# slcs-jsc/mptrac

Hardware: AMD Instinct MI355X
Metric: particle-steps/s (higher is better)
Workload: dtype f64

## Files before the change

### mptrac_amd/csrc/mphip_api.hip

```cpp
#include <hip/hip_runtime.h>
#include <dlfcn.h>
#include <unistd.h>

#include <algorithm>
#include <atomic>
#include <cmath>
#include <cstdio>
#include <cstring>
#include <string>
#include <mutex>
#include <thread>
#include <vector>

#include "mphip_kernels.hpp"
#include "mphip_metprep.hpp"
#include "mphip_regrid.hpp"
#include "mphip_detrend.hpp"

using namespace mphip;

namespace {

constexpr unsigned kAdv = MPHIP_MOD_TIMESTEPS | MPHIP_MOD_POSITION | MPHIP_MOD_ADVECT | MPHIP_MOD_POSITION2;
constexpr unsigned kAdvTurb = kAdv | MPHIP_MOD_DIFF_TURB;
constexpr unsigned kAdvDiff = kAdvTurb | MPHIP_MOD_DIFF_MESO;
constexpr unsigned kAdvTurbConvSedi = kAdvTurb | MPHIP_MOD_CONVECTION | MPHIP_MOD_SEDI;
constexpr unsigned kAdvDiffConvSedi = kAdvDiff | MPHIP_MOD_CONVECTION | MPHIP_MOD_SEDI;
constexpr unsigned kDiffConvSediOnly = MPHIP_MOD_TIMESTEPS | MPHIP_MOD_DIFF_TURB | MPHIP_MOD_DIFF_MESO | MPHIP_MOD_CONVECTION
  | MPHIP_MOD_SEDI | MPHIP_MOD_POSITION2;
constexpr unsigned kTailOnly = MPHIP_MOD_TIMESTEPS;
constexpr unsigned kBound = MPHIP_MOD_BOUND_COND | MPHIP_MOD_BOUND_COND2;
constexpr unsigned kParticleBits = 0x3fffu | MPHIP_MOD_ISOSURF | kBound | MPHIP_MOD_ISOSURF_INIT;

struct MetSlot {
  bool valid = false;
  double time = 0;
  float *f3[MPHIP_N3D] = {};
  float *f2[MPHIP_N2D] = {};
  bool has3[MPHIP_N3D] = {};
  bool has2[MPHIP_N2D] = {};
  std::vector<double> lon, lat, p;
  float ps11 = 0.f;
  double ps_min = -HUGE_VAL, pct_min = -HUGE_VAL;
  double ps_max = HUGE_VAL, pbl_min = -HUGE_VAL, pbl_max = HUGE_VAL, pel_min = -HUGE_VAL;
};

}

struct mphip_ctx {
  int device = 0;
  hipStream_t stream = nullptr;
  std::string err;
  std::mutex err_lock;

  mphip_ctl_t ctl;
  bool have_ctl = false;
  DevClim *d_clim = nullptr;
  bool have_clim = false;
  double *d_zm[MPHIP_NZM] = {};
  DevZm zm[MPHIP_NZM] = {};
  double *d_ts[MPHIP_NTR] = {};
  DevTracerSeries h_tracers = {};
  DevTracerSeries *d_tracers = nullptr;

  MetSlot slot[2];
  int flip = 0;
  MetSlot next;
  bool next_pending = false;
  hipStream_t copy_stream = nullptr;
  hipEvent_t next_ready = nullptr;
  hipEvent_t main_mark = nullptr;
  bool fuse_sort = true;
  const int *fused_perm = nullptr;
  bool fuse_quantities = true;
  bool fused_quantities = false;
  const int *fold_perm = nullptr;
  bool lazy_meteo = true;
  bool meteo_pending = false;
  bool pin_host_atm = false;
  std::vector<std::pair<uintptr_t, uintptr_t>> pinned;
  std::mutex pinned_lock;
  std::thread uploader;
  int uploader_rc = 0;
  std::atomic<bool> uploader_done{ false };
  std::string uploader_err;
  int nx = 0, ny = 0, npl = 0, coord_type = 0;
  int nml = 0;
  struct PackedGrids {
    float *wind = nullptr, *temp = nullptr, *h2o = nullptr;
    float *mlw = nullptr, *zl2 = nullptr, *pl2 = nullptr;
    f32x4 *mx = nullptr, *mx2 = nullptr;
    f32x4 *cloud = nullptr, *sfa = nullptr, *sfb = nullptr, *sfc = nullptr, *sfd = nullptr;
    f32x4 *cp2 = nullptr;
    int *ml_mono = nullptr;
    bool ml_monotonic = false;
    float *meso = nullptr;
    bool meso_valid = false;
    void release() {
      for (void *q : { (void *) wind, (void *) temp, (void *) h2o, (void *) mlw, (void *) zl2, (void *) pl2, (void *) mx,
                       (void *) mx2, (void *) cloud, (void *) sfa, (void *) sfb, (void *) sfc, (void *) sfd, (void *) cp2,
                       (void *) ml_mono, (void *) meso })
        if (q)
          (void) hipFree(q);
      *this = PackedGrids();
    }
  };
  PackedGrids pk, pk_next;
  bool pk_next_valid = false;
  std::vector<double> h_lon, h_lat, h_p;
  double *d_axes = nullptr;
  int lut_base = 0, lut_size = 0;
  size_t axes_bytes = 0;
  bool packed_dirty = true;

  long long np = 0, ip0 = 0, np_total = 0, cap = 0;
  int nq = 0;
  double *d_arr[4 + MPHIP_NQ_MAX] = {};
  double *d_alt[4 + MPHIP_NQ_MAX] = {};
  float *d_uvwp[3] = {};
  float *d_uvwp_alt[3] = {};
  double *d_dt = nullptr;
  double *d_dt_alt = nullptr;
  uint64_t rng_ctr = 0;
  double *d_iso = nullptr, *d_iso_alt = nullptr;
  int *d_kz = nullptr, *d_kz_alt = nullptr;
  double *d_iso_ts = nullptr, *d_iso_ps = nullptr;
  int iso_n = 0;

  int *d_ext = nullptr, *d_ext_alt = nullptr;
  bool ext_identity = true;
  int locality_interval = 60;
  double *d_rec = nullptr;
  size_t rec_cap = 0;
  bool grid_records = true;
  int chain_blocks = 0;
  double *h_sums = nullptr;
  size_t h_sums_cap = 0;
  double *d_grid_kernel = nullptr;
  double *d_ana_kernel = nullptr;
  size_t ana_kernel_cap = 0;
  uint32_t *d_marks = nullptr;
  size_t marks_cap = 0;
  int *d_slot_of = nullptr;
  size_t slot_of_cap = 0;
  uint32_t *d_ana_flags = nullptr;
  int grid_nk = 0;
  bool locality_zorder = false;
  int locality_tile = 0;
  int step_blocks = 8192;
  int step_blocks_multi = 32768;
  int xcd_map = 1;
  int big_grid = 0;
  int perm_records = 1;
  void *d_prec = nullptr;
  size_t prec_cap = 0;
  int multi_step = 64;
  bool fold_resort = true;
  bool force_generic = false;
  bool compact_depo = true;
  int sort_bits = 0;
  int steps_since_resort = 1 << 30;

  uint32_t *d_keys[2] = {};
  int *d_vals[2] = {};
  uint32_t *d_counts = nullptr;
  size_t counts_cap = 0;
  int sorted_buf = -1;
  int lds_tile = 0;
  bool emit_keys = true;
  unsigned char *d_depo_busy = nullptr;
  long long depo_busy_cap = 0;
  bool told_shortcuts_off = false;
  bool depo_busy_valid = false;
  bool sort_repair = true;
  bool ahead_priority = false;
  bool stored_is_sorted = false;
  long long sorted_n = 0;
  uint32_t *rep_sk = nullptr, *rep_mk[2] = {}, *rep_fk = nullptr, *rep_tiles = nullptr, *rep_nm = nullptr;
  int *rep_si = nullptr, *rep_mi[2] = {}, *rep_fv = nullptr;
  long long rep_cap = 0;
  bool sort_ahead = true;
  bool ahead_box = true;
  hipStream_t ahead_stream = nullptr;
  hipEvent_t ahead_mark = nullptr, ahead_done = nullptr;
  uint32_t *ahead_keys[2] = {};
  int *ahead_vals[2] = {};
  uint32_t *ahead_counts = nullptr;
  size_t ahead_counts_cap = 0;
  double *ahead_dt = nullptr;
  long long ahead_cap = 0;
  bool ahead_valid = false;
  double ahead_t = 0;
  int ahead_cur = 0;

  int *d_cell = nullptr;
  double *d_sums = nullptr;
  size_t sums_cap = 0;

  int *d_cnt = nullptr;
  double *d_chemgrid = nullptr;
  bool chemgrid_ok = false;
  double h2o2_low = 0;
  double *d_photo = nullptr;
  DevPhoto photo = {};
  bool photo_have[4] = {};
  RadioQnt radio = { { -1, -1, -1, -1, -1, -1 } };
  bool radio_on = false;
  bool rdepo_on = false;
  mphip_box_t rdepo_grid = {};
  double *d_rdepo_inv = nullptr;
// ... 77 lines not shown
    (void) hipFree(p);
}

int grid_for(long long n, int block = 256, int maxb = 8192) {
  long long b = (n + block - 1) / block;
  if (b < 1)
    b = 1;
  if (b > maxb)
    b = maxb;
  return (int) b;
}

DevAtm dev_atm(const mphip_ctx *c) {
  DevAtm a;
  a.time = c->d_arr[0];
  a.p = c->d_arr[1];
  a.lon = c->d_arr[2];
  a.lat = c->d_arr[3];
  for (int iq = 0; iq < MPHIP_NQ_MAX; iq++)
    a.q[iq] = iq < c->nq ? c->d_arr[4 + iq] : nullptr;
  a.up = c->d_uvwp[0];
  a.vp = c->d_uvwp[1];
  a.wp = c->d_uvwp[2];
  a.dt = c->d_dt;
  a.ext = c->ext_identity ? nullptr : c->d_ext;
  a.iso = c->d_iso;
  a.kz = c->d_kz;
  a.iso_ts = c->d_iso_ts;
  a.iso_ps = c->d_iso_ps;
  a.iso_n = c->iso_n;
  a.perm = c->fold_perm ? c->fold_perm : c->fused_perm;
  a.s_time = c->d_alt[0];
  a.s_p = c->d_alt[1];
  a.s_lon = c->d_alt[2];
  a.s_lat = c->d_alt[3];
  a.nq_perm = c->fold_perm || (c->fused_perm && c->fused_quantities) ? c->nq : 0;
  a.perm_all = c->fold_perm ? 1 : 0;
  a.s_up = c->d_uvwp_alt[0];
  a.s_vp = c->d_uvwp_alt[1];
  a.s_wp = c->d_uvwp_alt[2];
  a.s_dt = c->d_dt_alt;
  a.s_ext = c->d_ext_alt;
  a.ext_out = c->d_ext;
  for (int iq = 0; iq < MPHIP_NQ_MAX; iq++)
    a.s_q[iq] = iq < c->nq ? c->d_alt[4 + iq] : nullptr;
  a.np = c->np;
  a.ip0 = c->ip0;
  a.np_total = c->np_total;
  return a;
}

static bool weights_stay_inside(int coord_type, double first, double last) {
  return coord_type != 0 || (last - first >= 360.0 && first <= 0.0 && first >= -360.0);
}

DevMet dev_met(const mphip_ctx *c) {
  DevMet M;
  M.wind = c->pk.wind;
  M.temp = c->pk.temp;
  M.cloud = c->pk.cloud;
  M.mx = c->pk.mx;
  M.mx2 = c->pk.mx2;
  M.sfa = c->pk.sfa;
  M.sfb = c->pk.sfb;
  M.cp2 = c->pk.cp2;
  M.sfc = c->pk.sfc;
  M.sfd = c->pk.sfd;
  M.h2o = c->pk.h2o;
  M.mlw = c->pk.mlw;
  M.zl2 = c->pk.zl2;
  M.pl2 = c->pk.pl2;
  M.meso = c->pk.meso_valid ? c->pk.meso : nullptr;
  M.meso_nty = (c->ny + 2) / 4;
  M.ml_monotonic = c->pk.ml_monotonic ? 1 : 0;
  for (int t = 0; t < 2; t++) {
    M.zl[t] = c->slot[t ^ c->flip].f3[MPHIP_ZETAL];
    M.pll[t] = c->slot[t ^ c->flip].f3[MPHIP_PL];
  }
  M.npl = c->nml;
  M.axes = c->d_axes;
  M.lut_base = c->lut_base;
  M.lut_size = c->lut_size;
  M.lat_x0 = c->h_lat[0];
  M.lat_inv_dx = (c->ny - 1) / (c->h_lat[c->ny - 1] - c->h_lat[0]);
  M.nx = c->nx;
  M.ny = c->ny;
  M.np = c->npl;
  M.coord_type = c->coord_type;
  M.time0 = c->slot[0 ^ c->flip].time;
  M.time1 = c->slot[1 ^ c->flip].time;
  M.inv_dtime = 1.0 / (M.time1 - M.time0);
  double latmin = c->h_lat[0], latmax = c->h_lat[0];
  for (double v : c->h_lat) {
    latmin = std::min(latmin, v);
    latmax = std::max(latmax, v);
  }
  M.latmin = latmin;
  M.latmax = latmax;
  M.local = (std::fabs(c->h_lon[c->nx - 1] - c->h_lon[0] - 360.0) >= 0.01);
  const int my = (c->ny - 1) >> 1, mp = (c->npl - 1) >> 1;
  M.lat_ascending = c->h_lat[my] < c->h_lat[my + 1];
  M.p_ascending = c->h_p[mp] < c->h_p[mp + 1];
  M.lon_first = c->h_lon[0];
  M.lon_last = c->h_lon[c->nx - 1];
  M.inv_dlon0 = 1.0 / (c->h_lon[1] - c->h_lon[0]);
  M.lat_search_max = std::nextafter(latmax, -HUGE_VAL);
  M.p_min = *std::min_element(c->h_p.begin(), c->h_p.end());
  M.p_search_max = std::nextafter(*std::max_element(c->h_p.begin(), c->h_p.end()), -HUGE_VAL);
  M.p_cmp_off = M.p_ascending ? 1 : 0;
  M.p_step = M.p_ascending ? 1 : -1;
  M.ps11[0] = c->slot[0 ^ c->flip].ps11;
  M.ps11[1] = c->slot[1 ^ c->flip].ps11;
  M.ps_skip = std::min(c->slot[0].ps_min, c->slot[1].ps_min) - 1e-6;
  M.pct_skip = std::min(c->slot[0].pct_min, c->slot[1].pct_min) - 1e-6;
  {
    const double ps_lo = std::min(c->slot[0].ps_min, c->slot[1].ps_min), ps_hi = std::max(c->slot[0].ps_max, c->slot[1].ps_max);
    const double pbl_lo = std::min(c->slot[0].pbl_min, c->slot[1].pbl_min),
                 pbl_hi = std::max(c->slot[0].pbl_max, c->slot[1].pbl_max);
    auto p1_min = [&](double trans) {
      double lo = HUGE_VAL;
      for (double pbl : { pbl_lo, pbl_hi })
        for (double ps : { ps_lo, ps_hi })
          lo = std::min(lo, pbl - trans * (ps - pbl));
      return lo;
    };
    const bool known = std::isfinite(ps_lo) && std::isfinite(ps_hi) && std::isfinite(pbl_lo) && std::isfinite(pbl_hi);
    M.turb_skip = -HUGE_VAL;
    M.conv_skip = -HUGE_VAL;
    if (known && c->have_ctl) {
      const double b = std::min({ ps_lo, pbl_lo, p1_min(c->ctl.turb_pbl_trans) });
      M.turb_skip = b - 1e-6 * std::fabs(b) - 1e-6;
      double lo = ps_lo;
      if (c->ctl.conv_mix_pbl)
        lo = std::min(lo, p1_min(c->ctl.conv_pbl_trans));
      if (c->ctl.conv_cape >= 0)
        lo = std::min(lo, std::min(c->slot[0].pel_min, c->slot[1].pel_min));
      if (lo == lo)
        M.conv_skip = lo - 1e-6 * std::fabs(lo) - 1e-6;
    }
  }
  if (!weights_stay_inside(c->coord_type, c->h_lon[0], c->h_lon[c->nx - 1]))
    M.ps_skip = M.pct_skip = M.turb_skip = M.conv_skip = -HUGE_VAL;
  M.meso_dt = std::fabs(c->ctl.dt_mod);
  M.meso_r = 1 - 2 * M.meso_dt / c->ctl.dt_met;
  M.meso_r2 = std::sqrt(1 - M.meso_r * M.meso_r);
  if (!c->have_ctl || !(M.meso_dt > 0) || !std::isfinite(M.meso_r2))
    M.meso_dt = -1;
  return M;
}

size_t axes_lds_bytes(const mphip_ctx *c) {
  return c->axes_bytes;
}

int host_locate_irr(const std::vector<double> &xx, double x) {
  const int n = (int) xx.size();
  int lo = 0, hi = n - 1;
  int mid = (hi + lo) >> 1;
  if (xx[mid] < xx[mid + 1]) {
    while (hi > lo + 1) {
      mid = (hi + lo) >> 1;
      if (xx[mid] > x)
        hi = mid;
      else
        lo = mid;
    }
  } else {
    while (hi > lo + 1) {
      mid = (hi + lo) >> 1;
      if (xx[mid] <= x)
        hi = mid;
      else
        lo = mid;
    }
  }
  return lo;
}

int upload_axes(mphip_ctx *ctx) {
  const int nx = ctx->nx, ny = ctx->ny, np = ctx->npl;
  const size_t nd = 2 * (size_t) (nx + ny + np);
  std::vector<int16_t> lut;
  ctx->lut_base = ctx->lut_size = 0;
  const double pmin = *std::min_element(ctx->h_p.begin(), ctx->h_p.end());
  const double pmax = *std::max_element(ctx->h_p.begin(), ctx->h_p.end());
  if (pmin > 0 && std::isfinite(pmax) && np < 32000) {
    long long kmin, kmax;
    memcpy(&kmin, &pmin, 8);
    memcpy(&kmax, &pmax, 8);
    kmin >>= 45;
    kmax >>= 45;
    if (kmax - kmin + 1 <= 8192) {
      ctx->lut_base = (int) kmin;
      ctx->lut_size = (int) (kmax - kmin + 1);
      lut.resize((size_t) ctx->lut_size);
// ... 2570 lines not shown
    const int nx = ctl->chemgrid_nx, ny = ctl->chemgrid_ny, nz = ctl->chemgrid_nz;
    const double dz = (ctl->chemgrid_z1 - ctl->chemgrid_z0) / nz;
    const double dlon = (ctl->chemgrid_lon1 - ctl->chemgrid_lon0) / nx;
    const double dlat = (ctl->chemgrid_lat1 - ctl->chemgrid_lat0) / ny;
    std::vector<double> tab((size_t) nz + 2 * (size_t) ny + nx);
    double *press = tab.data(), *area = press + nz, *lon = area + ny, *lat = lon + nx;
    for (int iz = 0; iz < nz; iz++)
      press[iz] = kP0 * exp(-(ctl->chemgrid_z0 + dz * (iz + 0.5)) / kH0);
    for (int ix = 0; ix < nx; ix++)
      lon[ix] = ctl->chemgrid_lon0 + dlon * (ix + 0.5);
    for (int iy = 0; iy < ny; iy++) {
      lat[iy] = ctl->chemgrid_lat0 + dlat * (iy + 0.5);
      area[iy] = dlat * dlon * ((kRE * M_PI / 180.) * (kRE * M_PI / 180.)) * cos(lat[iy] * M_PI / 180.);
    }
    HIPCHK(hipSetDevice(ctx->device));
    HIPCHK(hipStreamSynchronize(ctx->stream));
    if (dev_alloc(ctx, &ctx->d_chemgrid, tab.size()))
      return 1;
    HIPCHK(hipMemcpy(ctx->d_chemgrid, tab.data(), tab.size() * sizeof(double), hipMemcpyHostToDevice));
    ctx->chemgrid_ok = true;
  }
  ctx->h2o2_low = pow(1. / kH2O2CorA, 1. / kH2O2CorB);
  ctx->ctl = *ctl;
  ctx->have_ctl = true;
  return 0;
}

int mphip_update_clim(mphip_ctx *ctx, int ntime, int nlat, const double *tropo_time, const double *tropo_lat,
                      const double *tropo, int ld) {
  if (!ctx || !tropo_time || !tropo_lat || !tropo)
    return fail(ctx, "null argument");
  if (ntime < 2 || ntime > 12 || nlat < 2 || nlat > 73 || ld < nlat)
    return fail(ctx, "tropopause climatology dimensions out of range");
  HIPCHK(hipSetDevice(ctx->device));
  DevClim h;
  memset(&h, 0, sizeof(h));
  h.ntime = ntime;
  h.nlat = nlat;
  for (int i = 0; i < ntime; i++)
    h.time[i] = tropo_time[i];
  for (int j = 0; j < nlat; j++)
    h.lat[j] = tropo_lat[j];
  for (int i = 0; i < ntime; i++)
    for (int j = 0; j < nlat; j++)
      h.tropo[i][j] = tropo[(size_t) i * ld + j];
  for (int i = 0; i + 1 < ntime; i++)
    h.inv_dtime[i] = 1.0 / (h.time[i + 1] - h.time[i]);
  for (int j = 0; j + 1 < nlat; j++)
    h.inv_dlat[j] = 1.0 / (h.lat[j + 1] - h.lat[j]);
  if (!ctx->d_clim)
    HIPCHK(hipMalloc((void **) &ctx->d_clim, sizeof(DevClim)));
  HIPCHK(hipMemcpyAsync(ctx->d_clim, &h, sizeof(DevClim), hipMemcpyHostToDevice, ctx->stream));
  HIPCHK(hipStreamSynchronize(ctx->stream));
  ctx->have_clim = true;
  return 0;
}

int mphip_update_clim_zm(mphip_ctx *ctx, int which, int ntime, int np, int nlat, const double *time, const double *p,
                         const double *lat, const double *vmr) {
  if (!ctx || which < 0 || which >= MPHIP_NZM)
    return fail(ctx, "bad argument");
  HIPCHK(hipSetDevice(ctx->device));
  if (flush_meteo(ctx))
    return 1;
  HIPCHK(hipStreamSynchronize(ctx->stream));
  dev_free(ctx->d_zm[which]);
  ctx->d_zm[which] = nullptr;
  memset(&ctx->zm[which], 0, sizeof(DevZm));
  if (ntime == 0)
    return 0;
  if (!time || !p || !lat || !vmr)
    return fail(ctx, "null argument");
  if (ntime < 2 || np < 2 || nlat < 2 || ntime > 4096 || np > 4096 || nlat > 4096)
    return fail(ctx, "climatology dimensions out of range");
  if (!(p[0] > p[1]))
    return fail(ctx, "Pressure data are not descending!");
  if (!(lat[0] < lat[1]))
    return fail(ctx, "Latitude data are not ascending!");
  const size_t nv = (size_t) ntime * (size_t) np * (size_t) nlat, n = (size_t) ntime + np + nlat + nv;
  double *d = nullptr;
  if (dev_alloc(ctx, &d, n))
    return 1;
  ctx->d_zm[which] = d;
  HIPCHK(hipMemcpy(d, time, (size_t) ntime * sizeof(double), hipMemcpyHostToDevice));
  HIPCHK(hipMemcpy(d + ntime, p, (size_t) np * sizeof(double), hipMemcpyHostToDevice));
  HIPCHK(hipMemcpy(d + ntime + np, lat, (size_t) nlat * sizeof(double), hipMemcpyHostToDevice));
  HIPCHK(hipMemcpy(d + ntime + np + nlat, vmr, nv * sizeof(double), hipMemcpyHostToDevice));
  DevZm &z = ctx->zm[which];
  z.time = d;
  z.p = d + ntime;
  z.lat = d + ntime + np;
  z.vmr = d + ntime + np + nlat;
  z.ntime = ntime;
  z.np = np;
  z.nlat = nlat;
  return 0;
}

int mphip_update_clim_photo(mphip_ctx *ctx, int np, int nsza, int no3c, const double *p, const double *sza,
                            const double *o3c, const double *const rate[MPHIP_NTR]) {
  if (!ctx)
    return 1;
  HIPCHK(hipSetDevice(ctx->device));
  if (flush_meteo(ctx))
    return 1;
  HIPCHK(hipStreamSynchronize(ctx->stream));
// ... 2043 lines not shown

int mphip_comm_query(mphip_ctx *ctx, int *nranks, int *rank) {
  if (!ctx || !nranks || !rank)
    return 1;
  *nranks = 0;
  *rank = 0;
  if (!ctx->comm)
    return 0;
  Rccl &R = rccl();
  RCCLCHK(R.CommCount(ctx->comm, nranks));
  RCCLCHK(R.CommUserRank(ctx->comm, rank));
  return 0;
}

int mphip_set_option(mphip_ctx *ctx, const char *name, double value) {
  if (!ctx || !name)
    return 1;
  if (strcmp(name, "locality_sort_interval") == 0) {
    if (value < 0)
      return fail(ctx, "locality_sort_interval must be >= 0");
    ctx->locality_interval = (int) value;
    return 0;
  }
  if (strcmp(name, "step_blocks") == 0 || strcmp(name, "step_blocks_multi") == 0) {
    if (value < 8 || value > 1048576)
      return fail(ctx, "step_blocks must be in 8 ... 1048576");
    (strcmp(name, "step_blocks") == 0 ? ctx->step_blocks : ctx->step_blocks_multi) = (int) value;
    return 0;
  }
  if (strcmp(name, "fuse_sort") == 0) {
    ctx->fuse_sort = value != 0;
    return 0;
  }
  if (strcmp(name, "lazy_meteo") == 0) {
    if (value == 0 && flush_meteo(ctx))
      return 1;
    ctx->lazy_meteo = value != 0;
    return 0;
  }
  if (strcmp(name, "pin_host_atm") == 0) {
    ctx->pin_host_atm = value != 0;
    return 0;
  }
  if (strcmp(name, "multi_step") == 0) {
    if (value < 0 || value > 4096)
      return fail(ctx, "multi_step must be in 0 ... 4096");
    ctx->multi_step = (int) value;
    return 0;
  }
  if (strcmp(name, "fold_resort") == 0) {
    ctx->fold_resort = value != 0;
    return 0;
  }
  if (strcmp(name, "fuse_sort_quantities") == 0) {
    ctx->fuse_quantities = value != 0;
    return 0;
  }
  if (strcmp(name, "perm_records") == 0) {
    ctx->perm_records = value != 0;
    return 0;
  }
  if (strcmp(name, "big_grid") == 0) {
    ctx->big_grid = value != 0;
    return 0;
  }
  if (strcmp(name, "derive_profile_phase") == 0) {
    if (value != 0 && value != 1 && value != 2 && value != 3)
      return fail(ctx, "derive_profile_phase must be 0 (kernels), 1 (uploads), 2 (downloads) or 3 (the weight table of "
                       "mphip_detrend_met)");
    ctx->prep_profile_phase = (int) value;
    return 0;
  }
  if (strcmp(name, "xcd_map") == 0) {
    ctx->xcd_map = value != 0;
    return 0;
  }
  if (strcmp(name, "generic_kernel") == 0) {
    ctx->force_generic = value != 0;
    return 0;
  }
  if (strcmp(name, "sort_bits") == 0) {
    if (!(value == 0 || (value >= 8 && value <= kRadixMaxBits)))
      return fail(ctx, "sort_bits must be 0 (automatic), 8, 9 or 10");
    ctx->sort_bits = (int) value;
    return 0;
  }
  if (strcmp(name, "mix_exchange_levels") == 0) {
    ctx->mix_exchange_levels = value != 0;
    return 0;
  }
  if (strcmp(name, "lds_tile") == 0) {
    if (value != 0 && (value < 64 || value > 2400))
      return fail(ctx, "lds_tile must be 0 or 64 ... 2400 cells");
    ctx->lds_tile = (int) value;
    return 0;
  }
  if (strcmp(name, "ahead_priority") == 0) {
    ctx->ahead_priority = value != 0;
    return 0;
  }
  if (strcmp(name, "emit_keys") == 0) {
    ctx->emit_keys = value != 0;
    return 0;
  }
  if (strcmp(name, "sort_repair") == 0) {
    ctx->sort_repair = value != 0;
// ... 252 lines not shown
```

### mptrac_amd/csrc/mphip_device.hpp

```cpp
#pragma once

#include <hip/hip_runtime.h>
#include <stdint.h>

#pragma GCC visibility push(default)
#include "../../include/mptrac_hip.h"
#pragma GCC visibility pop
#include "mphip_libm.h"
#include "mphip_libmtab.h"

namespace mphip {

struct LibmBlob {
  double log_tab[2 * MPHIP_LIBM_N];
  uint64_t exp_tab[2 * MPHIP_LIBM_N];
  double pow_tab[3 * MPHIP_LIBM_N];
};
static __device__ const LibmBlob g_libm = { { MPHIP_LIBM_LOG_TAB_INIT }, { MPHIP_LIBM_EXP_TAB_INIT }, { MPHIP_LIBM_POW_TAB_INIT } };
constexpr int kLibmLogExpDoubles = 4 * MPHIP_LIBM_N;
constexpr int kLibmDoubles = 7 * MPHIP_LIBM_N;

__device__ __forceinline__ const double *libm_tables() {
  return g_libm.log_tab;
}
// ... 57 lines not shown

constexpr double kG0 = 9.80665;
constexpr double kH0 = 7.0;
constexpr double kKB = 1.3806504e-23;
constexpr double kMA = 28.9644;
constexpr double kP0 = 1013.25;
constexpr double kRI = 8.3144598;
constexpr double kRA = 1e3 * kRI / kMA;
constexpr double kRE = 6367.421;
constexpr double kMAir = 4.8096e-26;
constexpr double kTRef = 298.15;
constexpr double kT0 = 273.15;
constexpr double kPi = 3.14159265358979323846;
constexpr double kSO2K1Ref = 1.23e-2, kSO2K1Temp = 2.01e3, kSO2K2Ref = 6e-8, kSO2K2Temp = 1.12e3;
constexpr double kWdTLiquid = kT0, kWdTIce = 238.15, kWdTLiquidBC = 270.;
constexpr double kEps = 18.01528 / kMA, kKappa = 0.286, kCpd = 1003.5, kKarman = 0.40;


struct DevMet {
  const float *wind;
  const float *temp;
  const f32x4 *cloud;
  const f32x4 *mx;
  const f32x4 *mx2;
  const f32x4 *sfa;
  const f32x4 *sfb;
  const f32x4 *cp2;
  const f32x4 *sfc;
  const f32x4 *sfd;
  const float *h2o;
  const float *mlw;
  const float *zl[2];
  const float *pll[2];
  const float *zl2, *pl2;
  int ml_monotonic;
  int npl;
  const double *axes;
  int nx, ny, np, coord_type;
  int lut_base, lut_size;
  double lat_x0, lat_inv_dx;
  double time0, time1;
  double inv_dtime;
  double latmin, latmax;
  int local;
  int lat_ascending, p_ascending;
  double lon_first, lon_last;
  double inv_dlon0;
  double lat_search_max;
  double p_min, p_search_max;
  int p_cmp_off, p_step;
  float ps11[2];
  double ps_skip, pct_skip;
  double turb_skip, conv_skip;
  double meso_dt, meso_r, meso_r2;
  const float *meso;
  int meso_nty;
};

struct DevAtm {
  double *time, *p, *lon, *lat;
  double *q[MPHIP_NQ_MAX];
  float *up, *vp, *wp;
  double *dt;
  const int *ext;
  double *iso;
  int *kz;
  const double *iso_ts, *iso_ps;
  int iso_n;
  const int *perm;
  const double *s_time, *s_p, *s_lon, *s_lat;
  const double *s_q[MPHIP_NQ_MAX];
  int nq_perm;
  int perm_all;
  const float *s_up, *s_vp, *s_wp;
  const double *s_dt;
  const int *s_ext;
  int *ext_out;
  long long np;
  long long ip0;
  long long np_total;
};

struct DevClim {
  int ntime, nlat;
  double time[12];
  double lat[73];
  double tropo[12][73];
  double inv_dtime[12];
  double inv_dlat[73];
};

struct Axes {
  const double *lon, *lat, *p;
  const double *inv_lon, *inv_lat, *inv_p;
  const short *p_lut;
};

__device__ __forceinline__ size_t axes_doubles(const DevMet &M) {
  return 2 * (size_t) (M.nx + M.ny + M.np);
}

__device__ __forceinline__ Axes load_axes(const DevMet &M, double *smem) {
  const size_t nd = axes_doubles(M);
  for (size_t i = threadIdx.x; i < nd; i += blockDim.x)
    smem[i] = M.axes[i];
  short *lut = (short *) (smem + nd);
  const short *glut = (const short *) (M.axes + nd);
  for (int i = threadIdx.x; i < M.lut_size; i += blockDim.x)
    lut[i] = glut[i];
  Axes A;
  A.lon = smem;
  A.lat = A.lon + M.nx;
  A.p = A.lat + M.ny;
  A.inv_lon = A.p + M.np;
  A.inv_lat = A.inv_lon + M.nx;
  A.inv_p = A.inv_lat + M.ny;
  A.p_lut = lut;
  return A;
}

#ifndef MPHIP_EXACT_DIV
#define MPHIP_EXACT_DIV 0
#endif
#ifndef MPHIP_WIND_CACHE
#define MPHIP_WIND_CACHE 1
#endif
#ifndef MPHIP_SETPRIO
#define MPHIP_SETPRIO 0
#endif


__device__ __forceinline__ double div_const(double x, double y, double inv_y) {
#if MPHIP_EXACT_DIV
  (void) inv_y;
  return x / y;
#else
  (void) y;
  return x * inv_y;
#endif
}


__device__ __forceinline__ double fdiv(double a, double b) {
#if MPHIP_EXACT_DIV
  return a / b;
#else
  double r = __builtin_amdgcn_rcp(b);
  r = __builtin_fma(__builtin_fma(-b, r, 1.0), r, r);
  const double q = a * r;
  return __builtin_fma(__builtin_fma(-b, q, a), r, q);
#endif
}

__device__ __forceinline__ double fsqrt(double x) {
#if MPHIP_EXACT_DIV
  return sqrt(x);
#else
  const double y = __builtin_amdgcn_rsq(x);
  double g = x * y, h = 0.5 * y;
  const double r = __builtin_fma(-h, g, 0.5);
  g = __builtin_fma(g, r, g);
  h = __builtin_fma(h, r, h);
  const double d = __builtin_fma(-g, g, x);
  g = __builtin_fma(d, h, g);
  return x == 0.0 ? x : g;
#endif
}


__device__ __forceinline__ double vmin(double a, double b) {
  double r;
  asm("v_min_f64 %0, %1, %2" : "=v"(r) : "v"(a), "v"(b));
  return r;
}

__device__ __forceinline__ double vmax(double a, double b) {
  double r;
  asm("v_max_f64 %0, %1, %2" : "=v"(r) : "v"(a), "v"(b));
  return r;
}

__device__ __forceinline__ double vmin_s(double a, double s) {
  double r;
  asm("v_min_f64 %0, %1, %2" : "=v"(r) : "v"(a), "s"(s));
  return r;
}

__device__ __forceinline__ double vmax_s(double a, double s) {
  double r;
  asm("v_max_f64 %0, %1, %2" : "=v"(r) : "v"(a), "s"(s));
  return r;
}

__device__ __forceinline__ int clamp0_s(int x, int hi) {
// ... 1069 lines not shown
  const double x2 = x * x;
  float sp, cp;
  {
    const double x3 = xs * x2;
    const double s1 = __builtin_fma(x2, -0x1.994eb3774cf24p-13, 0x1.1107605230bc4p-7);
    const double x7 = x3 * x2;
    const double sn = __builtin_fma(x3, -0x1.555545995a603p-3, xs);
    sp = (float) __builtin_fma(x7, s1, sn);
  }
  {
    const double x4 = x2 * x2;
    const double c2 = __builtin_fma(x2, 0x1.99343027bf8c3p-16, -0x1.6c087e89a359dp-10);
    const double c1 = __builtin_fma(x2, -0x1.ffffffd0c621cp-2, 0x1p0);
    const double x6 = x4 * x2;
    const double c = __builtin_fma(x4, 0x1.55553e1068f19p-5, c1);
    cp = __uint_as_float(__float_as_uint((float) __builtin_fma(x6, c2, c)) ^ ((uint32_t) (n & 2) << 30));
  }
  const bool even = (n & 1) == 0;
  sinv = even ? sp : cp;
  cosv = even ? cp : sp;
}

__device__ __forceinline__ float libm_sincosf(float y, int which) {
  float sv, cv;
  libm_sincosf_both(y, sv, cv);
  return which ? cv : sv;
}

__device__ __forceinline__ double u64_to_double(uint64_t r) {
  double hi;
  asm("v_cvt_f64_u32_e32 %0, %1" : "=v"(hi) : "v"((uint32_t) (r >> 32)));
  return __builtin_fma(hi, 0x1p32, (double) (uint32_t) r);
}

__device__ __forceinline__ void libm_log_unit_pair(const double *__restrict__ lt, double xa, double xb, double &la, double &lb) {
  const double ua = xa * 0x1p-64, ub = xb * 0x1p-64;
  const uint64_t ia = mphip_libm_bits(ua), ib = mphip_libm_bits(ub);
  la = mphip_libm_log_away(lt, ia);
  lb = mphip_libm_log_away(lt, ib);
  bool pa = mphip_libm_log_is_near_one(ia) | (xa == 0.0), pb = mphip_libm_log_is_near_one(ib) | (xb == 0.0);
  while (pa | pb) {
    const double x = pa ? ua : ub;
    const double v = x == 1.0 ? 0.0 : (x == 0.0 ? -__builtin_inf() : mphip_libm_log_near_one(x));
    if (pa) {
      la = v;
      pa = false;
    } else {
      lb = v;
      pb = false;
    }
  }
}

__device__ __forceinline__ void box_muller(double log_u, uint64_t rb, double &even, double &odd) {
  const double r = sqrt_rn(-2.0 * log_u);
  const float phif = (float) (u64_to_double(rb) * (2.0 * kPi * 0x1p-64));
  float sv, cv;
  libm_sincosf_both(phif, sv, cv);
  even = r * cv;
  odd = r * sv;
}

__device__ __forceinline__ void normal_pair_from(const double *__restrict__ ltab, uint64_t y, double &even, double &odd) {
  const uint64_t ra = squares_from(y), rb = squares_from(y + kSquaresKey);
  box_muller(libm_log(ltab, u64_to_double(ra) * 0x1p-64), rb, even, odd);
}

__device__ __forceinline__ void normal_two_pairs_from(const double *__restrict__ ltab, uint64_t y, double &ea, double &oa,
                                                      double &eb, double &ob) {
  double la, lb;
  libm_log_unit_pair(ltab, u64_to_double(squares_from(y)), u64_to_double(squares_from(y + 2 * kSquaresKey)), la, lb);
  asm volatile("" : "+v"(la), "+v"(lb));
  box_muller(la, squares_from(y + kSquaresKey), ea, oa);
  box_muller(lb, squares_from(y + 3 * kSquaresKey), eb, ob);
}

__device__ __forceinline__ void normal_pair(const double *__restrict__ ltab, uint64_t c0, uint64_t j2, double &even,
                                            double &odd) {
  normal_pair_from(ltab, (c0 + j2) * kSquaresKey, even, odd);
}

__device__ __forceinline__ void normal_triple(const double *__restrict__ ltab, uint64_t c0, uint64_t g, double &r0,
                                              double &r1, double &r2) {
  const uint64_t i0 = 3 * g;
  const bool odd = (i0 & 1) != 0;
  const uint64_t y = (c0 + (i0 & ~1ull)) * kSquaresKey;
  double ea, oa, eb, ob;
  normal_two_pairs_from(ltab, y, ea, oa, eb, ob);
  r0 = odd ? oa : ea;
  r1 = odd ? eb : oa;
  r2 = odd ? ob : eb;
}

#ifndef MPHIP_TURB_SHORTCUT
#define MPHIP_TURB_SHORTCUT 0
#endif
__device__ __forceinline__ double normal_third(const double *__restrict__ ltab, uint64_t c0, uint64_t g) {
  const uint64_t i0 = 3 * g;
  const uint64_t y = (c0 + (i0 & ~1ull)) * kSquaresKey;
  double eb, ob;
  normal_pair_from(ltab, y + 2 * kSquaresKey, eb, ob);
  return (i0 & 1) ? ob : eb;
}


struct Particle {
  double time, lon, lat, p, dt;
};

__device__ __forceinline__ double timestep_of(const mphip_ctl_t &ctl, const DevMet &M, const Axes &A, double time,
                                              double lon, double lat, double t) {
  const double dir = ctl.direction;
  double dt = 0.0;
  if (dir * (time - ctl.t_start) >= 0 && dir * (time - ctl.t_stop) <= 0 && dir * (time - t) < 0)
    dt = t - time;
  if (M.local && (lon <= A.lon[0] || lon >= A.lon[M.nx - 1] || lat <= M.latmin || lat >= M.latmax))
    dt = 0.0;
  return dt;
}

__device__ __forceinline__ void position(const DevMet &M, const Axes &A, Particle &P) {
  if (M.coord_type == 0) {
    double lon = fmod_trunc(P.lon, 360.);
    double lat = fmod_trunc(P.lat, 360.);
    while (lat < -90 || lat > 90) {
      if (lat > 90) {
        lat = 180 - lat;
        lon += 180;
      }
      if (lat < -90) {
        lat = -180 - lat;
        lon += 180;
      }
    }
    while (lon < -180)
      lon += 360;
    while (lon >= 180)
      lon -= 360;
    P.lon = lon;
    P.lat = lat;
  } else {
    const double x0 = A.lon[0], x1 = A.lon[M.nx - 1], y0 = A.lat[0], y1 = A.lat[M.ny - 1];
    P.lon = (x0 < x1) ? dmin(dmax(P.lon, x0), x1) : dmin(dmax(P.lon, x1), x0);
    P.lat = (y0 < y1) ? dmin(dmax(P.lat, y0), y1) : dmin(dmax(P.lat, y1), y0);
  }
  const double ptop = A.p[M.np - 1];
  if (P.p < ptop) {
    P.p = ptop * ptop / P.p;
  } else if (P.p > 300.) {
    const Stencil s = stencil_zero();
    SurfA c;
    load_sfa(M, s, c);
    const double ps = sfa_time_2d(c, s, time_weight(M, P.time), 0);
    if (P.p > ps)
// ... 1255 lines not shown
  const DegPerMetre dm = deg_per_metre(P.lat);
  double u = 0, v = 0, w = 0, um = 0, vm = 0, wm = 0;
  double x1 = P.lat;
#pragma unroll
  for (int i = 0; i < STAGES; i++) {
    if (STAGES == 2 && i == 1 && euler)
      break;
    double dts = 0.0, x0 = P.lon, x2 = P.p;
    x1 = P.lat;
    if (i > 0) {
      dts = (i == 3 ? 1.0 : 0.5) * dt;
      x0 = P.lon + dx2deg_k(dm, dts * u);
      x1 = P.lat + dy2deg_k(dts * v);
      x2 = P.p + dts * w;
    }
    Stencil s;
#if MPHIP_SETPRIO
    __builtin_amdgcn_s_setprio(MPHIP_SETPRIO);
#endif
    stencil_3d_fast(M, A, x2, x0, x1, s);
    load_wind_cached32<BIG>(M, s, wc, tile);
#if MPHIP_SETPRIO
    __builtin_amdgcn_s_setprio(0);
#endif
    hook(i);
    wind_cache_wait(wc);
    wind_uvw_fast(wc.c, s, time_weight(M, P.time + dts), u, v, w);
    if (STAGES == 4) {
      const double k = (i == 0 || i == 3) ? 1.0 / 6.0 : 2.0 / 6.0;
      um += k * u;
      vm += k * v;
      wm += k * w;
    } else {
      um = u;
      vm = v;
      wm = w;
    }
  }
  P.time += dt;
  if (STAGES == 2 && !euler) {
    const DegPerMetre dmid = deg_per_metre(x1);
    P.lon += dx2deg_k(dmid, dt * um);
  } else
    P.lon += dx2deg_k(dm, dt * um);
  P.lat += dy2deg_k(dt * vm);
  P.p += dt * wm;
}

template <class Hook>
__device__ __forceinline__ void advect_rk4_fast(const DevMet &M, const Axes &A, Particle &P, Hook &hook, WindCache &wc) {
  advect_fast<4>(M, A, P, hook, wc);
}

__device__ __forceinline__ void diff_turb_fast(const mphip_ctl_t &ctl, const DevMet &M, const Axes &A, const DevClim &C,
                                               Particle &P, uint64_t ctr, uint64_t g, const double *pre,
                                               const double *ltab) {
  const double wt = time_weight(M, P.time);
  const bool far = (P.p * 1.01 < M.turb_skip) & (wt >= 0.0) & (wt <= 1.0);
  double pbl = M.turb_skip, ps = M.turb_skip;
  const double lon0 = P.lon, lat0 = P.lat;
  if (!far) {
    Stencil s = stencil_zero();
    horiz_fast(M, A, P.lon, P.lat, s);
    SurfA c;
    load_pair_2d32(M.sfa, M, s, c);
    pbl = pair_time_2d_fast(c, s, wt, 1);
    if (ctl.turb_pbl_scheme > 0 && P.p >= pbl)
      return;
    ps = pair_time_2d_fast(c, s, wt, 0);
  }
  const double ptop = A.p[M.np - 1];

  const TropoTime tt = tropo_time(C, P.time);
  const double wpbl = pbl_weight(ctl, P.p, pbl, ps);
  double pt = tropo_pressure_at(ctl, C, tt, P.lat);
  const double wtrop = tropo_weight_pt(pt, P.p) * (1.0 - wpbl);
  const double wstrat = 1.0 - wpbl - wtrop;
  const double Kx = wpbl * ctl.turb_dx_pbl + wtrop * ctl.turb_dx_trop + wstrat * ctl.turb_dx_strat;
  const double Kz = wpbl * ctl.turb_dz_pbl + wtrop * ctl.turb_dz_trop + wstrat * ctl.turb_dz_strat;
  const double dt_abs = fabs(P.dt);

  double rs0 = 0, rs1 = 0, rs2;
  if (pre) {
    rs0 = pre[0];
    rs1 = pre[1];
    rs2 = pre[2];
  } else if (Kx > 0 || !MPHIP_TURB_SHORTCUT)
    normal_triple(ltab, ctr, g, rs0, rs1, rs2);
  else
    rs2 = normal_third(ltab, ctr, g);

  if (Kx > 0) {
    const double sigma_h = fsqrt(2.0 * Kx * dt_abs);
    const DegPerMetre dm = deg_per_metre(P.lat);
    P.lon += dx2deg_k(dm, rs0 * sigma_h);
    P.lat += dy2deg_k(rs1 * sigma_h);
    pt = tropo_pressure_at(ctl, C, tt, P.lat);
  }
  if (Kz > 0) {
    const double sigma_z = fsqrt(2.0 * Kz * dt_abs) * 1e-3;
    const double p_save = P.p;
    const double eps_km = 0.01;
    const double p_up = p_save + dz2dp(eps_km, p_save);
    const double p_dn = p_save + dz2dp(-eps_km, p_save);
    const double Kz_up = kz_blend(ctl, pt, vmax(ptop, vmin(ps, p_up)), pbl, ps);
    const double Kz_dn = kz_blend(ctl, pt, vmax(ptop, vmin(ps, p_dn)), pbl, ps);
    const double dKz_dz = div_const(Kz_up - Kz_dn, 2.0 * eps_km * 1e3, 1.0 / (2.0 * eps_km * 1e3));
    const double dlnrho_dz = -1.0 / (1e3 * kH0);
    const double w_drift = dKz_dz + Kz * dlnrho_dz;
    const double dz_drift = w_drift * dt_abs * 1e-3;
    const double dz_tot = rs2 * sigma_z + dz_drift;
    const double ptrial0 = p_save + dz2dp(dz_tot, p_save);
    double ptrial = ptrial0;
    bool at_surface = false;
    for (int iter = 0; iter < 10; iter++) {
      if (ptrial > ps) {
        at_surface = true;
        ptrial = ps * ps / ptrial;
      } else if (ptrial < ptop)
        ptrial = ptop * ptop / ptrial;
      else
        break;
    }
    if (far & (at_surface | !(ptrial <= ps))) {
      Stencil s = stencil_zero();
      horiz_fast(M, A, lon0, lat0, s);
      SurfA c;
      load_pair_2d32(M.sfa, M, s, c);
      ps = pair_time_2d_fast(c, s, wt, 0);
      ptrial = ptrial0;
      for (int iter = 0; iter < 10; iter++) {
        if (ptrial > ps)
          ptrial = ps * ps / ptrial;
        else if (ptrial < ptop)
          ptrial = ptop * ptop / ptrial;
        else
          break;
      }
    }
    P.p = dmax(ptop, dmin(ps, ptrial));
  }
}

template <class Corner>
__device__ __forceinline__ void meso_cell_sd(Corner corner, float sd[3]) {
#pragma clang fp contract(off)
  f32x2 mean_uv = { 0.f, 0.f }, sig_uv = { 0.f, 0.f };
  float mean_w = 0.f, sig_w = 0.f;
#pragma unroll
  for (int i = 0; i < 2; i++)
#pragma unroll
    for (int j = 0; j < 2; j++) {
      f32x4u r0, r1, r2;
      corner(i, j, r0, r1, r2);
      const f32x2 uv[2][2] = { { __builtin_shufflevector(r0, r0, 0, 1), __builtin_shufflevector(r0, r0, 2, 3) },
                               { __builtin_shufflevector(r1, r1, 2, 3), __builtin_shufflevector(r2, r2, 0, 1) } };
      const float ww[2][2] = { { r1[0], r1[1] }, { r2[2], r2[3] } };
#pragma unroll
      for (int k = 0; k < 2; k++)
#pragma unroll
        for (int t = 0; t < 2; t++) {
          mean_uv = mean_uv + uv[k][t];
          sig_uv = sig_uv + uv[k][t] * uv[k][t];
          mean_w = mean_w + ww[k][t];
          sig_w = sig_w + ww[k][t] * ww[k][t];
        }
    }
  const float mean[3] = { mean_uv[0], mean_uv[1], mean_w }, sig[3] = { sig_uv[0], sig_uv[1], sig_w };
#pragma unroll
  for (int q = 0; q < 3; q++) {
    const float m16 = mean[q] / 16.f;
    const float var = sig[q] / 16.f - m16 * m16;
    sd[q] = (var > 0 ? sqrtf(var) : 0.f);
  }
}

#ifndef MPHIP_MESO_TABLE
#define MPHIP_MESO_TABLE 1
#endif

struct MesoSd {
  float u, v, w;
};
__device__ __forceinline__ unsigned meso_off32(const DevMet &M, const Stencil &s) {
  const unsigned brick = __umul24(__umul24((unsigned) s.ix >> 2, (unsigned) M.meso_nty) + ((unsigned) s.iy >> 2),
                                  (unsigned) (M.np - 1)) + (unsigned) s.ip;
  return 12u * (16u * brick + (((unsigned) s.ix & 3u) << 2) + ((unsigned) s.iy & 3u));
}

template <bool STREAM = false, bool BIG = false>
__device__ __forceinline__ void diff_meso_fast(const mphip_ctl_t &ctl, const DevMet &M, const Axes &A, Particle &P,
                                               float &up, float &vp, float &wp, uint64_t ctr, uint64_t g,
                                               const double *pre, WindCache &wc, const double *ltab) {
// ... 324 lines not shown
```

### mptrac_amd/csrc/mphip_kernels.hpp

```cpp
#pragma once

#include <type_traits>
#include "mphip_device.hpp"

namespace mphip {



struct BoxGrid {
  double lon0, lon1, lat0, lat1, z0, z1;
  int nx, ny, nz;
};

constexpr int kMixMax = 8 + MPHIP_NRADIO;
struct MixSet {
  double *q[kMixMax];
  int n;
};

__device__ __forceinline__ int box_cell(const BoxGrid &G, double t0, double t1, double time, double lon, double lat,
                                        double p, const double *__restrict__ ens, long long i, int ngrid) {
  const double dz = (G.z1 - G.z0) / G.nz;
  const double dlon = (G.lon1 - G.lon0) / G.nx;
  const double dlat = (G.lat1 - G.lat0) / G.ny;
// ... 684 lines not shown
    };

    constexpr bool early = MPHIP_RNG_EARLY && !kRuntimeMask<CT> && (CT & MPHIP_MOD_ADVECT) && !(CT & kTwoStage) && !kLeanML<CT>;
    RngEarly pre;
    pre.mask = mask;
    pre.ctr_turb = c_turb;
    pre.ctr_meso = c_meso;
    pre.ctr_conv = c_conv;
    pre.g = early ? g_now() : 0;
    pre.ltab = ltab;

    constexpr bool lean = !kRuntimeMask<CT>;
    if (!kModelLevels<CT> && !(multi && MPHIP_MULTI_KEEP_WIND))
      wind_cache_reset(wc, CT != kMaskGeneric && (lean || !MPHIP_EXACT_DIV));
    if (mask & MPHIP_MOD_POSITION) {
      if (lean)
        position_fast(M, A, P);
      else
        position(M, A, P);
    }
    if (mask & MPHIP_MOD_ADVECT) {
      if (CT == kMaskGeneric && ctl.advect_vert_coord == 2) {
        advect_mlp(ctl, M, A, P);
      } else if (kModelLevels<CT> && ctl.advect_vert_coord == 2) {
        int kz = a.kz[i];
        advect_mlp_fast<MLCol>(ctl, M, A, P, kz);
        a.kz[i] = kz;
      } else if (CT == kMaskGeneric && (ctl.advect_vert_coord == 1 || ctl.advect_vert_coord == 3)) {
        const int qnt = ctl.advect_vert_coord == 1 ? ctl.qnt_zeta : ctl.qnt_eta;
        double zeta;
        advect_ml(ctl, M, A, P, zeta);
        a.q[qnt][i] = zeta;
      } else if (kModelLevels<CT>) {
        const int qnt = ctl.advect_vert_coord == 1 ? ctl.qnt_zeta : ctl.qnt_eta;
        double zeta;
        int kz = a.kz[i];
        advect_ml_fast<MLCol>(ctl, M, A, P, zeta, kz);
        a.kz[i] = kz;
        a.q[qnt][i] = zeta;
      } else if (lean && early)
        advect_rk4_fast(M, A, P, pre, wc);
      else if (lean && (CT & kTwoStage)) {
        NoHook none;
        advect_fast<2, kBig<CT>>(M, A, P, none, wc, ctl.advect == 1);
      } else if (lean) {
        NoHook none;
        advect_fast<4, kBig<CT>>(M, A, P, none, wc);
      } else
        advect(ctl, M, A, P, wc);
    }
    const unsigned opt = (lean && (CT & kGated)) ? (mask & S.mask & kOptionalModules) : (mask & kOptionalModules);
    if (opt & MPHIP_MOD_DIFF_TURB) {
      if (lean)
        diff_turb_fast(ctl, M, A, *clim, P, c_turb, g_now(), early ? pre.turb : nullptr, ltab);
      else
        diff_turb(ctl, M, A, *clim, P, c_turb, g_now(), early ? pre.turb : nullptr, ltab);
    }
#ifndef MPHIP_PBL_EMPTY
#define MPHIP_PBL_EMPTY 0
#endif
    constexpr bool lean_pbl = lean && (CT & kPblClosure) != 0 && !MPHIP_PBL_EMPTY;
    if (((CT == kMaskGeneric && (mask & MPHIP_MOD_DIFF_PBL)) || (lean_pbl && (S.mask & MPHIP_MOD_DIFF_PBL)))
        && !above_every_boundary_layer(M, P)) {
      const bool held = multi && (mask & MPHIP_MOD_DIFF_MESO);
      if (!held) {
        up = ld_state(&a.up[i]);
        vp = ld_state(&a.vp[i]);
        wp = ld_state(&a.wp[i]);
      }
      if constexpr (lean_pbl) {
        PblState st = { P.time, P.lon, P.lat, P.p, P.dt, up, vp, wp };
        st = diff_pbl_call(&M, A, st, c_pbl, g_now(), ltab);
        P.lon = st.lon;
        P.lat = st.lat;
        P.p = st.p;
        up = st.up;
        vp = st.vp;
        wp = st.wp;
        wind_cache_reset(wc, true);
      } else
        diff_pbl<false>(M, A, P, up, vp, wp, c_pbl, g_now(), ltab);
      if (!(store_once && held)) {
        st_state(&a.up[i], up);
        st_state(&a.vp[i], vp);
        st_state(&a.wp[i], wp);
      }
    }
    if (opt & MPHIP_MOD_DIFF_MESO) {
      if (!multi) {
        up = ld_state(&a.up[i]);
        vp = ld_state(&a.vp[i]);
        wp = ld_state(&a.wp[i]);
      }
      if (kGenericML<CT>)
        wind_cache_reset(wc, true);
      if (lean)
        diff_meso_fast<!(CT & MPHIP_MOD_ADVECT) || kLeanML<CT>, kBig<CT>>(ctl, M, A, P, up, vp, wp, c_meso, g_now(), early ? pre.meso : nullptr, wc, ltab);
      else
        diff_meso(ctl, M, A, P, up, vp, wp, c_meso, g_now(), early ? pre.meso : nullptr, wc, ltab);
      if (!store_once) {
        st_state(&a.up[i], up);
        st_state(&a.vp[i], vp);
        st_state(&a.wp[i], wp);
      }
    }
    if (lean) {
      if (opt & (MPHIP_MOD_CONVECTION | MPHIP_MOD_SEDI)) {
// ... 2599 lines not shown
```

Before: 14.64 billion.

## Add stratosphere fast path for turbulent diffusion using host-derived tropopause bound

Computes on the host a conservative pressure bound below the minimum climatological tropopause. When every lane in a wavefront is above it, diff_turb_fast uses the constant stratospheric Kz with no horizontal diffusion and skips the PBL and tropopause weighting, the Kz gradient stencil and two of the three normal draws. The bound is only enabled when turb_dx_strat is zero and the other settings are valid, so it is meant to stay exact. It also inlines the third-normal log computation with an asm barrier, and disables the path for big-grid kernels. Risks are extra wave-uniform branch divergence and reliance on the 0.8669 tropopause weighting factor.

```diff
diff --git a/mptrac_amd/csrc/mphip_api.hip b/mptrac_amd/csrc/mphip_api.hip
--- a/mptrac_amd/csrc/mphip_api.hip
+++ b/mptrac_amd/csrc/mphip_api.hip
@@ -56,6 +56,7 @@
   mphip_ctl_t ctl;
   bool have_ctl = false;
   DevClim *d_clim = nullptr;
+  DevClim h_clim = {};
   bool have_clim = false;
   double *d_zm[MPHIP_NZM] = {};
   DevZm zm[MPHIP_NZM] = {};
@@ -156,6 +157,7 @@
   size_t prec_cap = 0;
   int multi_step = 64;
   bool fold_resort = true;
+  bool turb_strat = true;
   bool force_generic = false;
   bool compact_depo = true;
   int sort_bits = 0;
@@ -339,6 +341,34 @@
 
 static bool weights_stay_inside(int coord_type, double first, double last) {
   return coord_type != 0 || (last - first >= 360.0 && first <= 0.0 && first >= -360.0);
+}
+
+static double clim_tropo_min(const DevClim &h) {
+  const double year = 365.25 * 86400.;
+  if (h.ntime < 2 || h.nlat < 2 || !(h.lat[0] <= -90.0 && h.lat[h.nlat - 1] >= 90.0))
+    return HUGE_VAL;
+  for (int i = 0; i + 1 < h.ntime; i++)
+    if (!(h.time[i] < h.time[i + 1]))
+      return HUGE_VAL;
+  for (int j = 0; j + 1 < h.nlat; j++)
+    if (!(h.lat[j] < h.lat[j + 1]))
+      return HUGE_VAL;
+  double lo = HUGE_VAL;
+  for (int i = 0; i + 1 < h.ntime; i++) {
+    const double w = h.time[i + 1] - h.time[i];
+    const double s0 = i == 0 ? std::min(0.0, (0.0 - h.time[0]) / w) : 0.0;
+    const double s1 = i + 2 == h.ntime ? std::max(1.0, (year - h.time[i]) / w) : 1.0;
+    for (int j = 0; j < h.nlat; j++) {
+      const double a = h.tropo[i][j], b = h.tropo[i + 1][j];
+      for (double s : { s0, s1 }) {
+        const double v = a + s * (b - a);
+        if (!(v == v))
+          return HUGE_VAL;
+        lo = std::min(lo, v);
+      }
+    }
+  }
+  return lo;
 }
 
 DevMet dev_met(const mphip_ctx *c) {
@@ -428,6 +458,19 @@
   }
   if (!weights_stay_inside(c->coord_type, c->h_lon[0], c->h_lon[c->nx - 1]))
     M.ps_skip = M.pct_skip = M.turb_skip = M.conv_skip = -HUGE_VAL;
+  M.strat_skip = -HUGE_VAL;
+  if (c->turb_strat && c->have_ctl && c->have_clim && M.turb_skip > -HUGE_VAL && c->ctl.met_coord_type == 0) {
+    const mphip_ctl_t &k = c->ctl;
+    bool ok = std::isfinite(k.turb_pbl_trans);
+    for (double v : { k.turb_dx_pbl, k.turb_dx_trop, k.turb_dx_strat, k.turb_dz_pbl, k.turb_dz_trop, k.turb_dz_strat })
+      ok = ok && std::isfinite(v) && v >= 0;
+    ok = ok && k.turb_dx_strat == 0;
+    const double b = 0.866877899 * clim_tropo_min(c->h_clim);
+    const double bound = b - 1e-6 * std::fabs(b) - 1e-6;
+    const double ptop = c->h_p[c->npl - 1] * 1.01;
+    if (ok && std::isfinite(bound) && ptop < bound && ptop < M.turb_skip)
+      M.strat_skip = bound;
+  }
   M.meso_dt = std::fabs(c->ctl.dt_mod);
   M.meso_r = 1 - 2 * M.meso_dt / c->ctl.dt_met;
   M.meso_r2 = std::sqrt(1 - M.meso_r * M.meso_r);
@@ -3104,6 +3147,7 @@
     HIPCHK(hipMalloc((void **) &ctx->d_clim, sizeof(DevClim)));
   HIPCHK(hipMemcpyAsync(ctx->d_clim, &h, sizeof(DevClim), hipMemcpyHostToDevice, ctx->stream));
   HIPCHK(hipStreamSynchronize(ctx->stream));
+  ctx->h_clim = h;
   ctx->have_clim = true;
   return 0;
 }
@@ -5253,6 +5297,10 @@
     ctx->fold_resort = value != 0;
     return 0;
   }
+  if (strcmp(name, "turb_strat") == 0) {
+    ctx->turb_strat = value != 0;
+    return 0;
+  }
   if (strcmp(name, "fuse_sort_quantities") == 0) {
     ctx->fuse_quantities = value != 0;
     return 0;
diff --git a/mptrac_amd/csrc/mphip_device.hpp b/mptrac_amd/csrc/mphip_device.hpp
--- a/mptrac_amd/csrc/mphip_device.hpp
+++ b/mptrac_amd/csrc/mphip_device.hpp
@@ -133,6 +133,7 @@
   float ps11[2];
   double ps_skip, pct_skip;
   double turb_skip, conv_skip;
+  double strat_skip;
   double meso_dt, meso_r, meso_r2;
   const float *meso;
   int meso_nty;
@@ -221,6 +222,14 @@
 #endif
 }
 
+
+__device__ __forceinline__ double mul_add(double x, double y, double c) {
+#if MPHIP_EXACT_DIV
+  return x * y + c;
+#else
+  return __builtin_fma(x, y, c);
+#endif
+}
 
 __device__ __forceinline__ double fdiv(double a, double b) {
 #if MPHIP_EXACT_DIV
@@ -1396,6 +1405,15 @@
   }
 }
 
+__device__ __forceinline__ double libm_log_unit(const double *__restrict__ lt, double xa) {
+  const double ua = xa * 0x1p-64;
+  const uint64_t ia = mphip_libm_bits(ua);
+  double la = mphip_libm_log_away(lt, ia);
+  if (mphip_libm_log_is_near_one(ia) | (xa == 0.0))
+    la = ua == 1.0 ? 0.0 : (ua == 0.0 ? -__builtin_inf() : mphip_libm_log_near_one(ua));
+  return la;
+}
+
 __device__ __forceinline__ void box_muller(double log_u, uint64_t rb, double &even, double &odd) {
   const double r = sqrt_rn(-2.0 * log_u);
   const float phif = (float) (u64_to_double(rb) * (2.0 * kPi * 0x1p-64));
@@ -1443,7 +1461,9 @@
   const uint64_t i0 = 3 * g;
   const uint64_t y = (c0 + (i0 & ~1ull)) * kSquaresKey;
   double eb, ob;
-  normal_pair_from(ltab, y + 2 * kSquaresKey, eb, ob);
+  double lb = libm_log_unit(ltab, u64_to_double(squares_from(y + 2 * kSquaresKey)));
+  asm volatile("" : "+v"(lb));
+  box_muller(lb, squares_from(y + 3 * kSquaresKey), eb, ob);
   return (i0 & 1) ? ob : eb;
 }
 
@@ -2805,93 +2825,111 @@
   advect_fast<4>(M, A, P, hook, wc);
 }
 
+__device__ __forceinline__ void turb_reflect(const DevMet &M, const Axes &A, Particle &P, double ptrial0, double ps,
+                                             double ptop, bool far, double lon0, double lat0, double wt) {
+  double ptrial = ptrial0;
+  bool at_surface = false;
+  for (int iter = 0; iter < 10; iter++) {
+    if (ptrial > ps) {
+      at_surface = true;
+      ptrial = ps * ps / ptrial;
+    } else if (ptrial < ptop)
+      ptrial = ptop * ptop / ptrial;
+    else
+      break;
+  }
+  if (far & (at_surface | !(ptrial <= ps))) {
+    Stencil s = stencil_zero();
+    horiz_fast(M, A, lon0, lat0, s);
+    SurfA c;
+    load_pair_2d32(M.sfa, M, s, c);
+    ps = pair_time_2d_fast(c, s, wt, 0);
+    ptrial = ptrial0;
+    for (int iter = 0; iter < 10; iter++) {
+      if (ptrial > ps)
+        ptrial = ps * ps / ptrial;
+      else if (ptrial < ptop)
+        ptrial = ptop * ptop / ptrial;
+      else
+        break;
+    }
+  }
+  P.p = dmax(ptop, dmin(ps, ptrial));
+}
+
+template <bool STRAT = true>
 __device__ __forceinline__ void diff_turb_fast(const mphip_ctl_t &ctl, const DevMet &M, const Axes &A, const DevClim &C,
                                                Particle &P, uint64_t ctr, uint64_t g, const double *pre,
                                                const double *ltab) {
   const double wt = time_weight(M, P.time);
   const bool far = (P.p * 1.01 < M.turb_skip) & (wt >= 0.0) & (wt <= 1.0);
-  double pbl = M.turb_skip, ps = M.turb_skip;
+  double ps = M.turb_skip;
   const double lon0 = P.lon, lat0 = P.lat;
-  if (!far) {
-    Stencil s = stencil_zero();
-    horiz_fast(M, A, P.lon, P.lat, s);
-    SurfA c;
-    load_pair_2d32(M.sfa, M, s, c);
-    pbl = pair_time_2d_fast(c, s, wt, 1);
-    if (ctl.turb_pbl_scheme > 0 && P.p >= pbl)
-      return;
-    ps = pair_time_2d_fast(c, s, wt, 0);
-  }
   const double ptop = A.p[M.np - 1];
-
-  const TropoTime tt = tropo_time(C, P.time);
-  const double wpbl = pbl_weight(ctl, P.p, pbl, ps);
-  double pt = tropo_pressure_at(ctl, C, tt, P.lat);
-  const double wtrop = tropo_weight_pt(pt, P.p) * (1.0 - wpbl);
-  const double wstrat = 1.0 - wpbl - wtrop;
-  const double Kx = wpbl * ctl.turb_dx_pbl + wtrop * ctl.turb_dx_trop + wstrat * ctl.turb_dx_strat;
-  const double Kz = wpbl * ctl.turb_dz_pbl + wtrop * ctl.turb_dz_trop + wstrat * ctl.turb_dz_strat;
-  const double dt_abs = fabs(P.dt);
-
-  double rs0 = 0, rs1 = 0, rs2;
-  if (pre) {
-    rs0 = pre[0];
-    rs1 = pre[1];
-    rs2 = pre[2];
-  } else if (Kx > 0 || !MPHIP_TURB_SHORTCUT)
-    normal_triple(ltab, ctr, g, rs0, rs1, rs2);
-  else
-    rs2 = normal_third(ltab, ctr, g);
-
-  if (Kx > 0) {
-    const double sigma_h = fsqrt(2.0 * Kx * dt_abs);
-    const DegPerMetre dm = deg_per_metre(P.lat);
-    P.lon += dx2deg_k(dm, rs0 * sigma_h);
-    P.lat += dy2deg_k(rs1 * sigma_h);
-    pt = tropo_pressure_at(ctl, C, tt, P.lat);
+  const double eps_km = 0.01;
+  const double dlnrho_dz = -1.0 / (1e3 * kH0);
+  double Kz, rs2, w_drift = 0.0;
+  if (STRAT && __all(far & (P.p * 1.01 < M.strat_skip) & (fabs(P.lat) <= 90.0))) {
+    Kz = ctl.turb_dz_strat;
+    w_drift = Kz * dlnrho_dz;
+    rs2 = pre ? pre[2] : normal_third(ltab, ctr, g);
+  } else {
+    double pbl = M.turb_skip;
+    if (!far) {
+      Stencil s = stencil_zero();
+      horiz_fast(M, A, P.lon, P.lat, s);
+      SurfA c;
+      load_pair_2d32(M.sfa, M, s, c);
+      pbl = pair_time_2d_fast(c, s, wt, 1);
+      if (ctl.turb_pbl_scheme > 0 && P.p >= pbl)
+        return;
+      ps = pair_time_2d_fast(c, s, wt, 0);
+    }
+
+    const TropoTime tt = tropo_time(C, P.time);
+    const double wpbl = pbl_weight(ctl, P.p, pbl, ps);
+    double pt = tropo_pressure_at(ctl, C, tt, P.lat);
+    const double wtrop = tropo_weight_pt(pt, P.p) * (1.0 - wpbl);
+    const double wstrat = 1.0 - wpbl - wtrop;
+    const double Kx = wpbl * ctl.turb_dx_pbl + wtrop * ctl.turb_dx_trop + wstrat * ctl.turb_dx_strat;
+    Kz = wpbl * ctl.turb_dz_pbl + wtrop * ctl.turb_dz_trop + wstrat * ctl.turb_dz_strat;
+
+    double rs0 = 0, rs1 = 0;
+    if (pre) {
+      rs0 = pre[0];
+      rs1 = pre[1];
+      rs2 = pre[2];
+    } else if (Kx > 0 || !MPHIP_TURB_SHORTCUT)
+      normal_triple(ltab, ctr, g, rs0, rs1, rs2);
+    else
+      rs2 = normal_third(ltab, ctr, g);
+
+    if (Kx > 0) {
+      const double sigma_h = fsqrt(2.0 * Kx * fabs(P.dt));
+      const DegPerMetre dm = deg_per_metre(P.lat);
+      P.lon += dx2deg_k(dm, rs0 * sigma_h);
+      P.lat += dy2deg_k(rs1 * sigma_h);
+      pt = tropo_pressure_at(ctl, C, tt, P.lat);
+    }
+    if (Kz > 0) {
+      const double p_up = P.p + dz2dp(eps_km, P.p);
+      const double p_dn = P.p + dz2dp(-eps_km, P.p);
+      const double Kz_up = kz_blend(ctl, pt, vmax(ptop, vmin(ps, p_up)), pbl, ps);
+      const double Kz_dn = kz_blend(ctl, pt, vmax(ptop, vmin(ps, p_dn)), pbl, ps);
+#if MPHIP_EXACT_DIV
+      w_drift = (Kz_up - Kz_dn) / (2.0 * eps_km * 1e3) + Kz * dlnrho_dz;
+#else
+      w_drift = __builtin_fma(Kz_up - Kz_dn, 1.0 / (2.0 * eps_km * 1e3), Kz * dlnrho_dz);
+#endif
+    }
   }
   if (Kz > 0) {
+    const double dt_abs = fabs(P.dt);
     const double sigma_z = fsqrt(2.0 * Kz * dt_abs) * 1e-3;
     const double p_save = P.p;
-    const double eps_km = 0.01;
-    const double p_up = p_save + dz2dp(eps_km, p_save);
-    const double p_dn = p_save + dz2dp(-eps_km, p_save);
-    const double Kz_up = kz_blend(ctl, pt, vmax(ptop, vmin(ps, p_up)), pbl, ps);
-    const double Kz_dn = kz_blend(ctl, pt, vmax(ptop, vmin(ps, p_dn)), pbl, ps);
-    const double dKz_dz = div_const(Kz_up - Kz_dn, 2.0 * eps_km * 1e3, 1.0 / (2.0 * eps_km * 1e3));
-    const double dlnrho_dz = -1.0 / (1e3 * kH0);
-    const double w_drift = dKz_dz + Kz * dlnrho_dz;
     const double dz_drift = w_drift * dt_abs * 1e-3;
-    const double dz_tot = rs2 * sigma_z + dz_drift;
-    const double ptrial0 = p_save + dz2dp(dz_tot, p_save);
-    double ptrial = ptrial0;
-    bool at_surface = false;
-    for (int iter = 0; iter < 10; iter++) {
-      if (ptrial > ps) {
-        at_surface = true;
-        ptrial = ps * ps / ptrial;
-      } else if (ptrial < ptop)
-        ptrial = ptop * ptop / ptrial;
-      else
-        break;
-    }
-    if (far & (at_surface | !(ptrial <= ps))) {
-      Stencil s = stencil_zero();
-      horiz_fast(M, A, lon0, lat0, s);
-      SurfA c;
-      load_pair_2d32(M.sfa, M, s, c);
-      ps = pair_time_2d_fast(c, s, wt, 0);
-      ptrial = ptrial0;
-      for (int iter = 0; iter < 10; iter++) {
-        if (ptrial > ps)
-          ptrial = ps * ps / ptrial;
-        else if (ptrial < ptop)
-          ptrial = ptop * ptop / ptrial;
-        else
-          break;
-      }
-    }
-    P.p = dmax(ptop, dmin(ps, ptrial));
+    const double dz_tot = mul_add(rs2, sigma_z, dz_drift);
+    turb_reflect(M, A, P, p_save + dz2dp(dz_tot, p_save), ps, ptop, far, lon0, lat0, wt);
   }
 }
 
diff --git a/mptrac_amd/csrc/mphip_kernels.hpp b/mptrac_amd/csrc/mphip_kernels.hpp
--- a/mptrac_amd/csrc/mphip_kernels.hpp
+++ b/mptrac_amd/csrc/mphip_kernels.hpp
@@ -760,7 +760,7 @@
     const unsigned opt = (lean && (CT & kGated)) ? (mask & S.mask & kOptionalModules) : (mask & kOptionalModules);
     if (opt & MPHIP_MOD_DIFF_TURB) {
       if (lean)
-        diff_turb_fast(ctl, M, A, *clim, P, c_turb, g_now(), early ? pre.turb : nullptr, ltab);
+        diff_turb_fast<!kBig<CT>>(ctl, M, A, *clim, P, c_turb, g_now(), early ? pre.turb : nullptr, ltab);
       else
         diff_turb(ctl, M, A, *clim, P, c_turb, g_now(), early ? pre.turb : nullptr, ltab);
     }
```

Result: faster. 14.92 billion, median of 6 (+2.0%).
